# jonasrothfuss/meta_learning_pacoh

Hardware: AMD Instinct MI355X
Metric: task-GP LML+grad evals/sec (n_ctx=64, d=4, 20 particles) (higher is better)
Workload: dtype f32; 1 GPU; PACOH-SVGD step as meta_fit runs it (hipGraph replay), cfg#3: 1024 tasks per GPU x 20 particles, n_ctx=64, d=4, NN(32,32) mean + NN(32,32) kernel (D=2534), task sharding + 1 all-reduce/step; parallelism=task-shard x1, finite=True, tasks_total=1024, particles=20, n_ctx=64, d=4

## Files before the change

### include/pacoh_gp.h

```cpp
#ifndef PACOH_GP_H
#define PACOH_GP_H

#include <stddef.h>
#include <stdint.h>

#ifdef __cplusplus
extern "C" {
#endif

#define PACOH_F32 0
#define PACOH_F64 1

#define PACOH_OK 0
#define PACOH_EINVAL (-1)
#define PACOH_ELIMIT (-2)
#define PACOH_EDTYPE (-3)
#define PACOH_ELAUNCH (-4)

#define PACOH_MEAN_ZERO 0
#define PACOH_MEAN_VECTOR 1
#define PACOH_MEAN_CONST 2

#define PACOH_MAX_FEATURES 16
#define PACOH_KERNEL_RBF 0
// ... 218 lines not shown
                           int bandwidth_ready, int dtype, void* stream);

typedef struct pacoh_active_tasks {
    const int32_t* n_act;
    const void* task_w;
} pacoh_active_tasks;
typedef struct pacoh_active_feed {
    const int32_t* nact_all;
    const void* mult_all;
    int32_t* n_act; void* task_w;
} pacoh_active_feed;
int pacoh_mlp2_fwd_active(const pacoh_active_tasks* act, const void* x, int x_div, const void* theta, long theta_stride, int P, int d_in,
                          const int32_t* hidden, int n_hidden, long off_a, int d_out_a, void* out_a, long off_b, int d_out_b,
                          void* out_b, void* workspace, void* stash, int B, int n, int dtype, void* stream);
int pacoh_mlp2_fwd_svgd_active(const pacoh_active_tasks* act, const void* x, int x_div, const void* theta, long theta_stride, int P,
                               int d_in, const int32_t* hidden, int n_hidden, long off_a, int d_out_a, void* out_a, long off_b,
                               int d_out_b, void* out_b, void* workspace, void* stash, int B, int n,
                               const void* svgd_X, void* svgd_workspace, int svgd_P, int svgd_D, int64_t* counter,
                               int dtype, void* stream);
int pacoh_gp_lml_fwdbwd_active(const pacoh_active_tasks* act, const void* z, int z_div, const void* mean, int mean_mode,
                               const void* y, int y_div, const void* lengthscale, const void* outputscale,
                               const void* noise, const int32_t* n_valid, const void* g_lml,
                               void* lml, void* d_z, void* d_mean, void* d_lengthscale,
                               void* d_outputscale, void* d_noise, int32_t* info,
                               int B, int P, int n, int f, int dtype, void* stream);
int pacoh_mlp2_bwd_hyper_active(const pacoh_active_tasks* act, const void* x, int x_div, const void* theta, long theta_stride, int P,
                                int d_in, const int32_t* hidden, int n_hidden, long off_a, int d_out_a, const void* g_a, long off_b,
                                int d_out_b, const void* g_b, void* d_theta, long d_theta_stride, int accumulate,
                                void* workspace, const void* stash, int B, int n,
                                int T, int off_ls, int f, int off_os, int off_noise, int off_const, const void* d_lengthscale,
                                const void* d_outputscale, const void* d_noise, const void* d_const, const void* lml, void* lik,
                                double lik_scale, const int32_t* info, int32_t* fail_flag, void* svgd_workspace, int svgd_P, int svgd_D,
                                const pacoh_adam_inline* opt, int dtype, void* stream);
int pacoh_step_begin_active(const pacoh_active_feed* feed, const int64_t* idx_all, int tb, const void* sc_all, int n_sc,
                            const void* aux_all, long n_aux, int64_t* counter, int32_t* ticket, void* sc_out, void* aux_out,
                            const void* x, const void* y, const int32_t* n_valid, void* out_x, void* out_y, int32_t* out_n_valid, int n, int d,
                            const void* theta, long theta_stride, int P, int off_ls, int f, int off_os, int off_noise, double noise_floor,
                            void* ls, void* os, void* noise, int advance, const void* svgd_X, void* svgd_workspace, int svgd_P, int svgd_D,
                            int dtype, void* stream);
int pacoh_svgd_update_next_active(const pacoh_active_feed* feed, void* X, const void* score, const void* prior_mean, const void* prior_std,
                                  double prior_factor, double bandwidth, int use_adam, double beta1, double beta2, void* exp_avg,
                                  void* exp_avg_sq, void* bw_out, void* workspace, int P, int D,
                                  const int64_t* counter, void* sc2, int n_sc, const int64_t* idx_all, int tb, const void* sc_all,
                                  const void* x, const void* y, const int32_t* n_valid, void* out_x, void* out_y,
                                  int32_t* out_n_valid, int n, int d,
                                  int off_ls, int f, int off_os, int off_noise, double noise_floor, void* ls, void* os, void* noise,
                                  int bandwidth_ready, int dtype, void* stream);
#define PACOH_DECLINED 1
#define PACOH_DISTINCT_MAX_DRAWS 4096
#define PACOH_DISTINCT_MAX_TASKS 8192
int pacoh_distinct_rows(const int64_t* idx, int64_t* rows, void* mult, int32_t* n_act, int k, int tb, int n_tasks, int dtype,
                        void* stream);
int pacoh_mlp_fused_split(int tiles_eff, int tiles_full, int wgs, int tpw_host);
int pacoh_mlp_fused_plan(int R, int P, int nets, int n_hidden, int bwd, int resident, int* tile_points, int* wgs, int* tiles_per_wg);

size_t pacoh_svgd_imq_workspace_bytes(int P, int D, int dtype);
int pacoh_svgd_phi_imq(const void* X, const void* score, double alpha, double beta, double bandwidth,
                       int neg, void* phi, void* h_out, void* workspace, int P, int D, int dtype,
                       void* stream);

int pacoh_adam_step(void* param, const void* grad, void* exp_avg, void* exp_avg_sq,
                    double lr, double beta1, double beta2, double eps, double weight_decay,
                    long step, long count, int dtype, void* stream);

int pacoh_adam_step_dev(void* param, const void* grad, void* exp_avg, void* exp_avg_sq, const void* scalars,
                        double beta1, double beta2, long count, int64_t* step_counter, void* loss_cum, const void* loss,
                        int dtype, void* stream);

size_t pacoh_vi_update_dev_workspace_bytes(int D, int dtype);
int pacoh_vi_update_dev(void* posterior, const void* eps, const void* theta, const void* score, const void* lik,
                        const void* log_q, const void* prior_mean, const void* prior_std, double prior_factor,
                        const void* scalars, double beta1, double beta2, void* exp_avg, void* exp_avg_sq, void* loss_out,
                        int64_t* step_counter, void* workspace, int S, int D, int dtype, void* stream);

int pacoh_axpy(void* y, const void* x, double alpha, long count, int dtype, void* stream);

int pacoh_vi_sample(const void* posterior, const void* eps, void* theta, void* log_q, int S, int D, int dtype, void* stream);
int pacoh_vi_grad(const void* posterior, const void* eps, const void* score, double prior_factor, void* grad,
                  int S, int D, int dtype, void* stream);

int pacoh_vi_sample_full(const void* posterior, const void* eps, void* theta, void* log_q, int S, int D, int dtype,
                         void* stream);
int pacoh_vi_grad_full(const void* posterior, const void* eps, const void* score, double prior_factor, void* grad,
                       int S, int D, int dtype, void* stream);

int pacoh_gather_tasks(const void* x, const void* y, const int32_t* n_valid, const int64_t* idx, void* out_x,
                       void* out_y, int32_t* out_n_valid, int Tb, int n, int d, int dtype, void* stream);

int pacoh_reduce_tasks(const void* in, void* out, double scale, int accumulate, int T, int P, int W,
                       int dtype, void* stream);

#define PACOH_MAX_QUANTILES 2048

int pacoh_mixture_cdf(const void* mu, const void* var, const void* value, void* cdf, double y_mean, double y_std, int T, int P,
                      int m, int dtype, void* stream);
int pacoh_mixture_icdf(const void* mu, const void* var, const void* quantile, void* out, double y_mean, double y_std, double lo,
                       double hi, double eps, int max_iter, int closed_form, int P, int m, int dtype, void* stream);
int pacoh_calib_error(const void* cdf, void* out, int T, int m, int dtype, void* stream);

size_t pacoh_mvn_factor_workspace_bytes(int B, int m, int dtype);
int pacoh_mvn_factor(const void* cov, void* L, int32_t* info, void* workspace, int B, int m, int dtype, void* stream);
int pacoh_mvn_sample(const void* L, const int32_t* info, const void* mu, const void* eps, const int32_t* order,
                     const int32_t* offsets, void* out, double y_mean, double y_std, int B, int m, int S, int dtype, void* stream);

int pacoh_map_persist_supported(int n, int d, int tb, int mean_mode, const int32_t* mean_hidden, int n_mean_hidden, int kernel_nn,
                                const int32_t* kernel_hidden, int n_kernel_hidden, int f, int dtype);
// ... 45 lines not shown
```

### meta_learning_pacoh_amd/_lib.py

```python
import ctypes
import os

import torch

_HERE = os.path.dirname(os.path.abspath(__file__))
LIB_PATH = os.environ.get('PACOH_LIB') or os.path.join(_HERE, 'lib', 'libpacoh_gp.so')

F32, F64 = 0, 1
MEAN_ZERO, MEAN_VECTOR, MEAN_CONST = 0, 1, 2
KERNEL_RBF, KERNEL_COSINE, KERNEL_SHIFT = 0, 1, 8
KERNEL_MATERN12, KERNEL_MATERN32, KERNEL_MATERN52 = 3, 4, 5


def _kf(f, kernel):
    return int(f) | (int(kernel) << KERNEL_SHIFT)
ERRORS = {-1: 'PACOH_EINVAL (bad argument)', -2: 'PACOH_ELIMIT (shape outside kernel limits)',
          -3: 'PACOH_EDTYPE', -4: 'PACOH_ELAUNCH (HIP launch failed)', -5: 'PACOH_ENOCOMM (librccl not loadable)'}
COMM_ID_BYTES = 128

_c = ctypes
_vp, _i, _l, _d, _sz = _c.c_void_p, _c.c_int, _c.c_long, _c.c_double, _c.c_size_t
_ip = _c.POINTER(_c.c_int32)

SIGNATURES = {
# ... 49 lines not shown
    'pacoh_step_select': (_i, [_vp, _i, _vp, _i, _vp, _l, _vp, _vp, _vp, _vp, _i, _vp]),
    'pacoh_scale_dev': (_i, [_vp, _vp, _l, _i, _vp]),
    'pacoh_distinct_rows': (_i, [_vp, _vp, _vp, _vp, _i, _i, _i, _i, _vp]),
    'pacoh_step_begin': (_i, [_vp, _i, _vp, _i, _vp, _l, _vp, _vp, _vp, _vp, _vp, _vp, _vp, _vp, _vp, _vp, _i, _i,
                              _vp, _l, _i, _i, _i, _i, _i, _d, _vp, _vp, _vp, _i, _vp, _vp, _i, _i, _i, _vp]),
    'pacoh_step_begin_vi': (_i, [_vp, _i, _vp, _i, _vp, _l, _vp, _vp, _vp, _vp, _vp, _vp, _vp, _vp, _vp, _vp, _i, _i,
                                 _vp, _i, _i, _vp, _vp, _i, _i, _i, _i, _d, _vp, _vp, _vp, _i, _i, _vp]),
    'pacoh_svgd_update_dev_workspace_bytes': (_sz, [_i, _i, _i]),
    'pacoh_svgd_update_dev': (_i, [_vp, _vp, _vp, _vp, _d, _d, _i, _vp, _d, _d, _vp, _vp, _vp, _vp, _i, _i, _i, _vp, _i, _vp]),
    'pacoh_svgd_dist_advance': (_i, [_vp, _vp, _i, _i, _vp, _i, _vp]),
    'pacoh_svgd_update_next': (_i, [_vp, _vp, _vp, _vp, _d, _d, _i, _d, _d, _vp, _vp, _vp, _vp, _i, _i,
                                    _vp, _vp, _i, _vp, _i, _vp, _vp, _vp, _vp, _vp, _vp, _vp, _i, _i,
                                    _i, _i, _i, _i, _d, _vp, _vp, _vp, _i, _i, _vp]),
    'pacoh_prior_logprob_grad': (_i, [_vp, _vp, _vp, _vp, _vp, _d, _i, _i, _i, _vp]),
    'pacoh_prior_score_dev': (_i, [_vp, _vp, _vp, _vp, _d, _vp, _i, _i, _i, _vp]),
    'pacoh_svgd_workspace_bytes': (_sz, [_i, _i, _i]),
    'pacoh_svgd_phi': (_i, [_vp, _vp, _d, _i, _vp, _vp, _vp, _i, _i, _i, _vp]),
    'pacoh_svgd_update': (_i, [_vp, _vp, _vp, _vp, _d, _d, _i, _d, _d, _d, _d, _l, _vp, _vp, _vp, _vp, _vp, _i, _i, _i, _vp]),
    'pacoh_svgd_imq_workspace_bytes': (_sz, [_i, _i, _i]),
    'pacoh_svgd_phi_imq': (_i, [_vp, _vp, _d, _d, _d, _i, _vp, _vp, _vp, _i, _i, _i, _vp]),
    'pacoh_adam_step': (_i, [_vp, _vp, _vp, _vp, _d, _d, _d, _d, _d, _l, _l, _i, _vp]),
    'pacoh_adam_step_dev': (_i, [_vp, _vp, _vp, _vp, _vp, _d, _d, _l, _vp, _vp, _vp, _i, _vp]),
    'pacoh_vi_update_dev_workspace_bytes': (_sz, [_i, _i]),
    'pacoh_vi_update_dev': (_i, [_vp, _vp, _vp, _vp, _vp, _vp, _vp, _vp, _d, _vp, _d, _d, _vp, _vp, _vp, _vp, _vp, _i, _i, _i, _vp]),
    'pacoh_axpy': (_i, [_vp, _vp, _d, _l, _i, _vp]),
    'pacoh_vi_sample': (_i, [_vp, _vp, _vp, _vp, _i, _i, _i, _vp]),
    'pacoh_vi_grad': (_i, [_vp, _vp, _vp, _d, _vp, _i, _i, _i, _vp]),
    'pacoh_vi_sample_full': (_i, [_vp, _vp, _vp, _vp, _i, _i, _i, _vp]),
    'pacoh_vi_grad_full': (_i, [_vp, _vp, _vp, _d, _vp, _i, _i, _i, _vp]),
    'pacoh_gather_tasks': (_i, [_vp, _vp, _vp, _vp, _vp, _vp, _vp, _i, _i, _i, _i, _vp]),
    'pacoh_reduce_tasks': (_i, [_vp, _vp, _d, _i, _i, _i, _i, _i, _vp]),
    'pacoh_mixture_cdf': (_i, [_vp, _vp, _vp, _vp, _d, _d, _i, _i, _i, _i, _vp]),
    'pacoh_mixture_icdf': (_i, [_vp, _vp, _vp, _vp, _d, _d, _d, _d, _d, _i, _i, _i, _i, _i, _vp]),
    'pacoh_calib_error': (_i, [_vp, _vp, _i, _i, _i, _vp]),
    'pacoh_mvn_factor_workspace_bytes': (_sz, [_i, _i, _i]),
    'pacoh_mvn_factor': (_i, [_vp, _vp, _vp, _vp, _i, _i, _i, _vp]),
    'pacoh_mvn_sample': (_i, [_vp, _vp, _vp, _vp, _vp, _vp, _vp, _d, _d, _i, _i, _i, _i, _vp]),
    'pacoh_map_persist_supported': (_i, [_i, _i, _i, _i, _ip, _i, _i, _ip, _i, _i, _i]),
    'pacoh_map_persist': (_i, [_vp, _vp, _vp, _i, _vp, _vp, _vp, _i, _i, _vp, _i, _vp, _i, _i, _i, _i, _ip, _i, _i, _i, _ip, _i, _i,
                               _i, _i, _i, _d, _ip, _ip, _i, _d, _d, _vp, _vp, _vp, _i, _vp]),
    'pacoh_map_task_workspace_bytes': (_sz, [_i, _i, _i, _i, _i, _ip, _i, _i, _ip, _i, _i, _i, _i]),
    'pacoh_map_task_setup': (_i, [_vp, _i, _i, _i, _i, _i, _i, _ip, _i, _i, _i, _ip, _i, _i, _vp, _sz, _i, _vp]),
    'pacoh_svgd_task_workspace_bytes': (_sz, [_i, _i, _i, _i, _i, _i, _ip, _i, _i, _ip, _i, _i, _i, _i]),
    'pacoh_svgd_task_setup': (_i, [_i, _i, _i, _i, _i, _i, _i, _ip, _i, _i, _i, _ip, _i, _i, _vp, _sz, _i, _vp]),
    'pacoh_svgd_task_step': (_i, [_vp, _l, _i, _vp, _vp, _vp, _i, _i, _i, _i, _i, _ip, _i, _i, _i, _ip, _i, _i, _vp, _vp, _vp, _i, _i, _i,
                                  _vp, _l, _vp, _d, _vp, _vp, _sz, _vp, _vp, _i, _vp, _i, _i, _vp]),
    'pacoh_map_task_step': (_i, [_vp, _l, _vp, _vp, _vp, _i, _i, _i, _i, _i, _ip, _i, _i, _i, _ip, _i, _i, _vp, _vp, _vp, _i, _i, _i,
                                 _vp, _l, _vp, _d, _vp, _vp, _sz, _vp, _i, _vp]),
    'pacoh_comm_unique_id': (_i, [_vp]),
    'pacoh_comm_init': (_i, [_vp, _i, _i, _c.POINTER(_vp)]),
    'pacoh_allreduce_sum': (_i, [_vp, _l, _i, _vp, _vp]),
    'pacoh_comm_destroy': (_i, [_vp]),
    'pacoh_mlp_fused_split': (_i, [_i, _i, _i, _i]),
    'pacoh_mlp_fused_plan': (_i, [_i, _i, _i, _i, _i, _i, _ip, _ip, _ip]),
}
for _name in ('pacoh_mlp2_fwd', 'pacoh_mlp2_fwd_svgd', 'pacoh_gp_lml_fwdbwd', 'pacoh_mlp2_bwd_hyper', 'pacoh_step_begin',
              'pacoh_svgd_update_next'):
    SIGNATURES[_name + '_active'] = (_i, [_vp] + SIGNATURES[_name][1])

_lib = None
ABI_VERSION = 14


def load_library():
    global _lib
    if _lib is None:
        if not os.path.exists(LIB_PATH):
            raise RuntimeError(
                'libpacoh_gp.so not found at %s -- build it with `python -c "import __graft_entry__ as g; '
                'g.build()"` (needs hipcc). There is no CPU fallback for the PACOH GP path.' % LIB_PATH)
        lib = ctypes.CDLL(LIB_PATH)
        for name, (res, args) in SIGNATURES.items():
            if not hasattr(lib, name):
                raise RuntimeError('libpacoh_gp.so does not export %s (stale build?)' % name)
            fn = getattr(lib, name)
            fn.restype, fn.argtypes = res, args
        if lib.pacoh_abi_version() != ABI_VERSION:
            raise RuntimeError('%s has ABI version %d, this binding expects %d (stale build?)'
                               % (LIB_PATH, lib.pacoh_abi_version(), ABI_VERSION))
        _lib = lib
    return _lib


class ActiveTasks(ctypes.Structure):
    _fields_ = [('n_act', _vp), ('task_w', _vp)]


class ActiveFeed(ctypes.Structure):
    _fields_ = [('nact_all', _vp), ('mult_all', _vp), ('n_act', _vp), ('task_w', _vp)]


def _active_tasks(active):
    if active is None:
        return None
    n_act, task_w = active
    assert n_act.dtype == torch.int32 and n_act.is_cuda and task_w.is_cuda
    return ActiveTasks(n_act.data_ptr(), task_w.data_ptr())


def _active_feed(feed):
    if not getattr(feed, 'dedup', False):
        return None
    return ActiveFeed(feed.nact_all.data_ptr(), feed.mult_all.data_ptr(), feed.nact.data_ptr(), feed.mult.data_ptr())


def _active_call(lib, name, act, *args):
# ... 1334 lines not shown
```

### meta_learning_pacoh_amd/csrc/mlp_fused.hip

```cpp
#include "common.h"
#include "hyper_tail.h"
#include "step_tail.h"
#include "mlp_fused_split.h"
#include <stdlib.h>

namespace pacoh {

using f32x4 = __attribute__((ext_vector_type(4))) float;

constexpr int FMAXNH = 4;
constexpr int LWH = 36;
constexpr int HBLK = 32 * LWH + 32;
constexpr int F_OFF_W1 = 0;
constexpr int F_OFF_B1 = 128;
constexpr int F_OFF_H = 160;
__host__ __device__ constexpr int f_off_out(int nh) { return F_OFF_H + (nh - 1) * HBLK; }
__host__ __device__ constexpr int f_welems(int nh) { return f_off_out(nh) + 68; }
__host__ __device__ constexpr int f_dnet_max(int nh) { return 32 * 5 + (nh - 1) * 32 * 33 + 2 * 33; }
__host__ __device__ constexpr bool bwd_wg_slab(int nh) { return nh <= 2; }
constexpr int TSTRIDE = 4;
constexpr int TSTAGE = 6;
constexpr int TLD = 17;
__host__ __device__ constexpr int tskew(int k) { return 12 * (k & 1) + 32 * (k >> 1); }
constexpr int TRS = 320;

struct FusedNet {
    long theta_off;
    float* out;
    const float* g_out;
    float* slab;
    float* stash;
    int d_out, D_net;
};

struct FusedArgs {
    const float* x; int x_div;
    const float* theta; long theta_stride;
    FusedNet net[2];
    int P, n, R;
    int d_in, nh;
    int h[FMAXNH];
    int tiles_per_wg;
    int n_stash;
    int nblk;
    int tail_z;
    SvgdDistTail<float> sv;
    const float* bw_d2; float* bw_out; int bw_P;
    long* adv_counter;
    const int32_t* n_act;
    int tiles;
};

__device__ __forceinline__ void fused_live_rows(const FusedArgs& a, int tp, int& R, int& tpw) {
    R = a.R; tpw = a.tiles_per_wg;
    if (!a.n_act) return;
    const int live = *a.n_act * a.n;
    if (live < R) R = live;
    tpw = fused_split_tiles((R + tp - 1) / tp, a.tiles, (int)gridDim.x, tpw);
}

__device__ __forceinline__ long stash_off(const FusedArgs& a, int p, int blk, int slot, int fb, int lane) {
    return (((((long)p * a.nblk + blk) * a.n_stash + slot) * 2 + fb) << 8) + (lane << 2);
}

__device__ __forceinline__ f32x4 fmfma(float a, float b, f32x4 c) {
    return __builtin_amdgcn_mfma_f32_16x16x4f32(a, b, c, 0, 0, 0);
}

constexpr float TSC = 2.8853900817779268f, INV_TSC = 0.34657359027997264f;
__device__ __forceinline__ float tanh_pre(float a) {
    return fmaf(-2.0f, __builtin_amdgcn_rcpf(1.0f + __builtin_amdgcn_exp2f(a)), 1.0f);
}

template <int NH>
__device__ void fused_load_weights(float* wl, const float* __restrict__ th, const FusedArgs& a, int d_out) {
    for (int q = threadIdx.x; q < f_welems(NH); q += blockDim.x) wl[q] = 0.0f;
    __syncthreads();
    int src = 0;
    const int h0 = a.h[0], d_in = a.d_in;
    for (int q = threadIdx.x; q < h0; q += blockDim.x) wl[F_OFF_B1 + q] = TSC * th[q];
    for (int q = threadIdx.x; q < h0 * d_in; q += blockDim.x) { const int o = q / d_in, k = q - o * d_in; wl[F_OFF_W1 + o * 4 + k] = TSC * th[h0 + q]; }
    src += h0 * (d_in + 1);
    int prev = h0;
#pragma unroll
    for (int l = 1; l < NH; ++l) {
        const int hl = a.h[l];
        float* dst = wl + F_OFF_H + (l - 1) * HBLK;
        for (int q = threadIdx.x; q < hl; q += blockDim.x) dst[32 * LWH + q] = TSC * th[src + q];
        for (int q = threadIdx.x; q < hl * prev; q += blockDim.x) { const int o = q / prev, k = q - o * prev; dst[o * LWH + k] = TSC * th[src + hl + q]; }
        src += hl * (prev + 1);
        prev = hl;
    }
    float* dst = wl + f_off_out(NH);
    for (int q = threadIdx.x; q < d_out; q += blockDim.x) dst[64 + q] = th[src + q];
    for (int q = threadIdx.x; q < d_out * prev; q += blockDim.x) { const int o = q / prev, k = q - o * prev; dst[o * 32 + k] = th[src + d_out + q]; }
    __syncthreads();
}

template <int PB, bool BWD>
__device__ __forceinline__ long stage_tile(const FusedArgs& a, const FusedNet& nt, int p, int row0, float* st, int lane, int R) {
    long orow = -1;
    if (lane < 16 * PB) {
        const int row = row0 + lane;
        const bool valid = row < R;
        const int rr = valid ? row : R - 1;
        const int t = (int)((unsigned)rr / (unsigned)a.n), i = rr - t * a.n;
        const int bi = t * a.P + p;
        const int xb = a.x_div == 1 ? bi : (int)((unsigned)bi / (unsigned)a.x_div);
        const float* xq = a.x + ((long)xb * a.n + i) * (long)a.d_in;
        float4 xv;
        xv.x = xq[0];
        xv.y = a.d_in > 1 ? xq[1] : 0.0f;
        xv.z = a.d_in > 2 ? xq[2] : 0.0f;
        xv.w = a.d_in > 3 ? xq[3] : 0.0f;
        *reinterpret_cast<float4*>(st + lane * TSTRIDE) = xv;
        const long o = (long)bi * a.n + i;
        if (BWD) {
            const float* gq = nt.g_out + o * nt.d_out;
            st[16 * PB * TSTRIDE + lane] = valid ? gq[0] : 0.0f;
            st[16 * PB * (TSTRIDE + 1) + lane] = (valid && nt.d_out > 1) ? gq[1] : 0.0f;
        }
        orow = valid ? o : -1;
    }
    asm volatile("" ::: "memory");
    return orow;
}

template <int PB>
__device__ __forceinline__ void f_layer1(const float* wl, const float* st, int r, int g, f32x4 (&H)[2][PB]) {
    float bx[PB];
#pragma unroll
    for (int pb = 0; pb < PB; ++pb) bx[pb] = st[(pb * 16 + r) * TSTRIDE + g];
#pragma unroll
    for (int fb = 0; fb < 2; ++fb) {
        f32x4 bias;
#pragma unroll
        for (int s = 0; s < 4; ++s) bias[s] = wl[F_OFF_B1 + fb * 16 + 4 * g + s];
        const float aw = wl[F_OFF_W1 + (fb * 16 + r) * 4 + g];
#pragma unroll
        for (int pb = 0; pb < PB; ++pb) {
            f32x4 acc = fmfma(aw, bx[pb], bias);
#pragma unroll
            for (int s = 0; s < 4; ++s) acc[s] = tanh_pre(acc[s]);
            H[fb][pb] = acc;
        }
    }
}

template <int PB>
__device__ __forceinline__ void f_hidden(const float* W, int r, int g, const f32x4 (&IN)[2][PB], f32x4 (&OUT)[2][PB]) {
#pragma unroll
    for (int ob = 0; ob < 2; ++ob) {
        f32x4 bias;
#pragma unroll
        for (int s = 0; s < 4; ++s) bias[s] = W[32 * LWH + ob * 16 + 4 * g + s];
#pragma unroll
        for (int pb = 0; pb < PB; ++pb) OUT[ob][pb] = bias;
#pragma unroll
        for (int kb = 0; kb < 2; ++kb) {
            const float4 aw = *reinterpret_cast<const float4*>(W + (ob * 16 + r) * LWH + kb * 16 + 4 * g);
#pragma unroll
            for (int pb = 0; pb < PB; ++pb) {
                f32x4 acc = OUT[ob][pb];
                acc = fmfma(aw.x, IN[kb][pb][0], acc); acc = fmfma(aw.y, IN[kb][pb][1], acc);
                acc = fmfma(aw.z, IN[kb][pb][2], acc); acc = fmfma(aw.w, IN[kb][pb][3], acc);
                OUT[ob][pb] = acc;
            }
        }
#pragma unroll
        for (int pb = 0; pb < PB; ++pb)
#pragma unroll
            for (int s = 0; s < 4; ++s) OUT[ob][pb][s] = tanh_pre(OUT[ob][pb][s]);
    }
}

template <int PB>
__device__ __forceinline__ void f_delta(const float* W, int r, int g, const f32x4 (&DOUT)[2][PB], f32x4 (&HIN)[2][PB]) {
#pragma unroll
// ... 22 lines not shown
    f32x4 o;
#pragma unroll
    for (int s = 0; s < 4; ++s) scr[wr + s * TLD] = v[s];
    asm volatile("" ::: "memory");
#pragma unroll
    for (int q = 0; q < 4; ++q) o[q] = scr[rd + q];
    asm volatile("" ::: "memory");
    return o;
}

__device__ __forceinline__ void f_wgrad(f32x4& acc, const f32x4& Ap, const f32x4& Bp) {
    acc = fmfma(Ap[0], Bp[0], acc); acc = fmfma(Ap[1], Bp[1], acc);
    acc = fmfma(Ap[2], Bp[2], acc); acc = fmfma(Ap[3], Bp[3], acc);
}

__device__ __forceinline__ void stash_st(const f32x4& v, f32x4* q) {
    __builtin_nontemporal_store(v, q);
}
__device__ __forceinline__ f32x4 stash_ld(const f32x4* q) {
    return *q;
}

template <int PB>
__device__ __forceinline__ void stash_put(const FusedArgs& a, const FusedNet& nt, int p, int blk0, int slot, int lane,
                                          const f32x4 (&H)[2][PB]) {
#pragma unroll
    for (int pb = 0; pb < PB; ++pb)
#pragma unroll
        for (int fb = 0; fb < 2; ++fb)
            stash_st(H[fb][pb], reinterpret_cast<f32x4*>(nt.stash + stash_off(a, p, blk0 + pb, slot, fb, lane)));
}

template <int PB>
__device__ __forceinline__ void stash_get(const FusedArgs& a, const FusedNet& nt, int p, int blk0, int slot, int lane,
                                          f32x4 (&H)[2][PB], int R) {
#pragma unroll
    for (int pb = 0; pb < PB; ++pb) {
        const bool in = (blk0 + pb) * 16 < R;
#pragma unroll
        for (int fb = 0; fb < 2; ++fb)
            H[fb][pb] = in ? stash_ld(reinterpret_cast<const f32x4*>(nt.stash + stash_off(a, p, blk0 + pb, slot, fb, lane)))
                           : f32x4{0.f, 0.f, 0.f, 0.f};
    }
}

template <int NH, int PB, int MINW>
__global__ void __launch_bounds__(256, MINW) mlp_fused_fwd_kernel(FusedArgs a) {
    __shared__ __attribute__((aligned(16))) float wl[f_welems(NH)];
    __shared__ __attribute__((aligned(16))) float stage[4][16 * PB * TSTAGE];
    if (a.tail_z > 0 && (int)blockIdx.z == a.tail_z) {
        svgd_dist_tail<float>(a.sv, (int)(blockIdx.y * gridDim.x + blockIdx.x), (int)(gridDim.x * gridDim.y));
        return;
    }
    int R, tpw;
    fused_live_rows(a, 16 * PB, R, tpw);
    const FusedNet& nt = a.net[blockIdx.z];
    const int p = blockIdx.y;
    fused_load_weights<NH>(wl, a.theta + (long)p * a.theta_stride + nt.theta_off, a, nt.d_out);
    const int lane = threadIdx.x & 63, wave = __builtin_amdgcn_readfirstlane(threadIdx.x >> 6);
    const int r = lane & 15, g = lane >> 4;
    float* st = stage[wave];
    const float* wo = wl + f_off_out(NH);
    float w3r[2][2][4];
#pragma unroll
    for (int o = 0; o < 2; ++o)
#pragma unroll
        for (int fb = 0; fb < 2; ++fb)
#pragma unroll
            for (int s = 0; s < 4; ++s) w3r[o][fb][s] = wo[o * 32 + fb * 16 + 4 * g + s];
    const float b30 = wo[64], b31 = wo[65];
    constexpr int TP = 16 * PB;
    for (int tl = wave; tl < tpw; tl += 4) {
        const int row0 = (blockIdx.x * tpw + tl) * TP;
        if (row0 >= R) break;
        const long orow_l = stage_tile<PB, false>(a, nt, p, row0, st, lane, R);
        f32x4 HA[2][PB], HB[2][PB];
        const int blk0 = row0 >> 4;
        const int ns = nt.stash ? a.n_stash : 0;
        f_layer1<PB>(wl, st, r, g, HA);
        if (ns >= NH) stash_put<PB>(a, nt, p, blk0, 0, lane, HA);
#pragma unroll
        for (int l = 1; l < NH; ++l) {
            if (l & 1) f_hidden<PB>(wl + F_OFF_H + (l - 1) * HBLK, r, g, HA, HB);
            else f_hidden<PB>(wl + F_OFF_H + (l - 1) * HBLK, r, g, HB, HA);
            if (l >= NH - ns) stash_put<PB>(a, nt, p, blk0, l - (NH - ns), lane, (l & 1) ? HB : HA);
        }
        const f32x4 (&HL)[2][PB] = ((NH - 1) & 1) ? HB : HA;
#pragma unroll
        for (int pb = 0; pb < PB; ++pb) {
            float v0 = 0.f, v1 = 0.f;
#pragma unroll
            for (int fb = 0; fb < 2; ++fb)
#pragma unroll
                for (int s = 0; s < 4; ++s) { v0 = fmaf(w3r[0][fb][s], HL[fb][pb][s], v0); v1 = fmaf(w3r[1][fb][s], HL[fb][pb][s], v1); }
            v0 += __shfl_xor(v0, 16, 64); v0 += __shfl_xor(v0, 32, 64);
            v1 += __shfl_xor(v1, 16, 64); v1 += __shfl_xor(v1, 32, 64);
            const long orow = __shfl(orow_l, pb * 16 + r, 64);
            if (g == 0 && orow >= 0) {
                nt.out[orow * nt.d_out] = v0 + b30;
                if (nt.d_out > 1) nt.out[orow * nt.d_out + 1] = v1 + b31;
            }
        }
    }
}

template <int NH, int PB, int MINW>
__global__ void __launch_bounds__(256, MINW) mlp_fused_bwd_kernel(FusedArgs a) {
    constexpr int L_WL = (f_welems(NH) + 3) & ~3, L_ST = 4 * 16 * PB * TSTAGE, L_TS = 4 * 2 * TRS;
    constexpr int L_RED = bwd_wg_slab(NH) ? 4 * f_dnet_max(NH) : 0;
    constexpr int L_ALL = (L_WL + L_ST + L_TS) > L_RED ? (L_WL + L_ST + L_TS) : L_RED;
    __shared__ __attribute__((aligned(16))) float lds[L_ALL];
    if (a.tail_z > 0 && (int)blockIdx.z == a.tail_z) {
        if (blockIdx.x == 0 && blockIdx.y == 0) {
            if (a.bw_out) svgd_bandwidth_block<float>(a.bw_d2, a.bw_P, a.bw_out);
            if (a.adv_counter && threadIdx.x == 0) *a.adv_counter += 1;
        }
        return;
    }
    int R, tpw;
    fused_live_rows(a, 16 * PB, R, tpw);
    float* wl = lds;
    const FusedNet& nt = a.net[blockIdx.z];
    const int p = blockIdx.y;
    fused_load_weights<NH>(wl, a.theta + (long)p * a.theta_stride + nt.theta_off, a, nt.d_out);
    const int lane = threadIdx.x & 63, wave = __builtin_amdgcn_readfirstlane(threadIdx.x >> 6);
    const int r = lane & 15, g = lane >> 4;
    float* st = lds + L_WL + wave * (16 * PB * TSTAGE);
    float* sc0 = lds + L_WL + L_ST + wave * (2 * TRS);
    float* sc1 = sc0 + TRS;
    const int twr = 4 * TLD * g + tskew(g) + r, trd = TLD * r + tskew(r >> 2) + 4 * g;
    const float* wo = wl + f_off_out(NH);

    f32x4 aW[NH > 1 ? NH - 1 : 1][2][2] = {};
    float aBh[NH > 1 ? NH - 1 : 1][2] = {};
    float aW1[2][4] = {}, aB1[2] = {};
    f32x4 aWoT[2][2] = {};
    float aBoT[2] = {};

    constexpr int TP = 16 * PB;
    for (int tl = wave; tl < tpw; tl += 4) {
        const int row0 = (blockIdx.x * tpw + tl) * TP;
        if (row0 >= R) break;
        stage_tile<PB, true>(a, nt, p, row0, st, lane, R);
        f32x4 H[NH][2][PB];
        const int blk0 = row0 >> 4;
        const int ns = nt.stash ? a.n_stash : 0;
#pragma unroll
        for (int l = NH - 1; l >= 0; --l)
            if (l >= NH - ns) stash_get<PB>(a, nt, p, blk0, l - (NH - ns), lane, H[l], R);
        if (ns < NH) f_layer1<PB>(wl, st, r, g, H[0]);
#pragma unroll
        for (int l = 1; l < NH; ++l)
            if (l < NH - ns) f_hidden<PB>(wl + F_OFF_H + (l - 1) * HBLK, r, g, H[l - 1], H[l]);
        {
// ... 181 lines not shown
    return (tiles + best_tpw - 1) / best_tpw;
}

static int fused_n_stash(int n_hidden) { return n_hidden > 1 ? n_hidden - 1 : 0; }
static int fused_nblk(int B, int P, int n) { return 4 * (int)(((long)(B / P) * n + 63) / 64); }

size_t mlp_fused_stash_bytes(int B, int P, int n, int n_hidden, int nets) {
    return (size_t)nets * P * fused_nblk(B, P, n) * fused_n_stash(n_hidden) * 2 * 256 * sizeof(float);
}

static void fused_fill(FusedArgs& a, const void* x, int x_div, const void* theta, long theta_stride, int P, int d_in,
                       const int32_t* hidden, int n_hidden, int B, int n, const void* stash, int nets) {
    a.x = (const float*)x; a.x_div = x_div; a.theta = (const float*)theta; a.theta_stride = theta_stride;
    a.P = P; a.n = n; a.R = (B / P) * n; a.d_in = d_in; a.nh = n_hidden;
    for (int l = 0; l < FMAXNH; ++l) a.h[l] = l < n_hidden ? hidden[l] : 0;
    a.n_stash = stash ? fused_n_stash(n_hidden) : 0;
    a.nblk = fused_nblk(B, P, n);
    const size_t per_net = (size_t)P * a.nblk * a.n_stash * 2 * 256;
    for (int k = 0; k < 2; ++k) a.net[k].stash = (a.n_stash > 0 && k < nets) ? (float*)stash + k * per_net : nullptr;
}

static int fused_fwd_tpw(int tiles, int P, int nets) {
    int pick = 4;
    double best = 1e30;
    for (int tpw = 4; tpw <= 32; tpw *= 2) {
        const long waves = (long)((tiles + tpw - 1) / tpw) * P * nets * 4;
        const double cost = (double)((waves + 1023) / 1024) * (tpw / 4 + 0.5);
        if (cost <= best * 1.02 || tpw == 4) { if (cost < best) best = cost; pick = tpw; }
    }
    return pick;
}

constexpr int BWD_MINW = 3;
constexpr int BWD_MINW_PB2 = 2;
#define PACOH_FUSED_DISPATCH(KERNEL, nh, pb, M)                                                          \
    do {                                                                                                 \
        if (pb == 4) {                                                                                   \
            if (nh == 1) { M((KERNEL<1, 4, BWD_MINW>)); } else if (nh == 2) { M((KERNEL<2, 4, BWD_MINW>)); }  \
            else if (nh == 3) { M((KERNEL<3, 4, 1>)); } else { M((KERNEL<4, 4, 1>)); }                    \
        } else {                                                                                         \
            if (nh == 1) { M((KERNEL<1, 2, BWD_MINW_PB2>)); } else if (nh == 2) { M((KERNEL<2, 2, BWD_MINW_PB2>)); }            \
            else if (nh == 3) { M((KERNEL<3, 2, 2>)); } else { M((KERNEL<4, 2, 2>)); }                    \
        }                                                                                                \
    } while (0)

int mlp_fused_fwd(const void* x, int x_div, const void* theta, long theta_stride, int P, int d_in, const int32_t* hidden,
                  int n_hidden, int nets, const long* off, const int* d_out, void* const* out, void* stash, int B, int n,
                  hipStream_t s, const SvgdDistTail<float>* tail, bool* tail_taken, const int32_t* n_act) {
    FusedArgs a = {};
    fused_fill(a, x, x_div, theta, theta_stride, P, d_in, hidden, n_hidden, B, n, stash, nets);
    for (int k = 0; k < nets; ++k) { a.net[k].theta_off = off[k]; a.net[k].out = (float*)out[k]; a.net[k].d_out = d_out[k]; }
    const int pb = fused_fwd_pb(a.R, P, nets);
    const int tiles = (a.R + 16 * pb - 1) / (16 * pb);
    a.n_act = n_act; a.tiles = tiles;
    a.tiles_per_wg = fused_fwd_tpw(tiles, P, nets);
    const int wgs = (tiles + a.tiles_per_wg - 1) / a.tiles_per_wg;
    if (tail && (long)wgs * P * 2 < (long)tail->P * (tail->P + 1) / 2) tail = nullptr;
    if (tail_taken) *tail_taken = tail != nullptr;
    if (tail) { a.tail_z = nets; a.sv = *tail; }
#define PACOH_LAUNCH_FWD(K) hipLaunchKernelGGL((K), dim3(wgs, P, nets + (tail ? 1 : 0)), dim3(256), 0, s, a)
    if (pb == 4) {
        if (n_hidden == 1) PACOH_LAUNCH_FWD((mlp_fused_fwd_kernel<1, 4, 4>)); else if (n_hidden == 2) PACOH_LAUNCH_FWD((mlp_fused_fwd_kernel<2, 4, 4>));
        else if (n_hidden == 3) PACOH_LAUNCH_FWD((mlp_fused_fwd_kernel<3, 4, 4>)); else PACOH_LAUNCH_FWD((mlp_fused_fwd_kernel<4, 4, 4>));
    } else {
        if (n_hidden == 1) PACOH_LAUNCH_FWD((mlp_fused_fwd_kernel<1, 2, 4>)); else if (n_hidden == 2) PACOH_LAUNCH_FWD((mlp_fused_fwd_kernel<2, 2, 4>));
        else if (n_hidden == 3) PACOH_LAUNCH_FWD((mlp_fused_fwd_kernel<3, 2, 4>)); else PACOH_LAUNCH_FWD((mlp_fused_fwd_kernel<4, 2, 4>));
    }
#undef PACOH_LAUNCH_FWD
    return launch_status();
}

struct FusedBwdPlan { int pb, chunks, tiles_per_wg; };

static FusedBwdPlan fused_bwd_plan(int R, int P, int nets, int n_hidden, int resident_given = 0) {
    FusedBwdPlan pl;
    pl.pb = fused_bwd_pb(n_hidden, R, P, nets);
    static int resident[FMAXNH + 1][2] = {};
    int res = resident_given;
    if (res <= 0) {
        int& cached = resident[n_hidden][pl.pb == 4];
        if (cached == 0) {
#define PACOH_OCC(K) cached = resident_wgs(K)
            PACOH_FUSED_DISPATCH(mlp_fused_bwd_kernel, n_hidden, pl.pb, PACOH_OCC);
#undef PACOH_OCC
        }
        res = cached;
    }
    const int tp = 16 * pl.pb;
    pl.chunks = fused_chunks(R, P, nets, tp, res, 0.4 * 64 / tp);
    const int tiles = (R + tp - 1) / tp;
    pl.tiles_per_wg = (tiles + pl.chunks - 1) / pl.chunks;
    return pl;
}

size_t mlp_fused_bwd_workspace(int B, int P, int n, int d_in, const int32_t* hidden, int n_hidden, int d_out, int nets) {
    const FusedBwdPlan pl = fused_bwd_plan((B / P) * n, P, nets, n_hidden);
    return (size_t)pl.chunks * (bwd_wg_slab(n_hidden) ? 1 : 4) * P * fused_dnet(d_in, hidden, n_hidden, d_out) * sizeof(float);
}

int mlp_fused_bwd(const void* x, int x_div, const void* theta, long theta_stride, int P, int d_in, const int32_t* hidden,
                  int n_hidden, int nets, const long* off, const int* d_out, const void* const* g_out, void* d_theta,
                  long d_theta_stride, int accumulate, void* workspace, const void* stash, int B, int n, hipStream_t s,
                  const HyperBwdArgs<float>* tail, long col_base) {
    FusedArgs a = {};
    fused_fill(a, x, x_div, theta, theta_stride, P, d_in, hidden, n_hidden, B, n, stash, nets);
    const FusedBwdPlan pl = fused_bwd_plan(a.R, P, nets, n_hidden);
    a.tiles_per_wg = pl.tiles_per_wg;
    a.n_act = tail ? tail->n_act : nullptr; a.tiles = (a.R + 16 * pl.pb - 1) / (16 * pl.pb);
    float* ws = (float*)workspace;
    SlabReduce sr[2] = {};
    int wmax = 0;
    for (int k = 0; k < nets; ++k) {
        a.net[k].theta_off = off[k]; a.net[k].g_out = (const float*)g_out[k]; a.net[k].d_out = d_out[k];
        a.net[k].D_net = fused_dnet(d_in, hidden, n_hidden, d_out[k]);
        a.net[k].slab = ws;
        sr[k].in = ws; sr[k].out = (float*)d_theta + off[k]; sr[k].Wd = a.net[k].D_net; sr[k].col0 = (int)(col_base + off[k]);
        ws += (size_t)pl.chunks * (bwd_wg_slab(n_hidden) ? 1 : 4) * P * a.net[k].D_net;
        if (a.net[k].D_net > wmax) wmax = a.net[k].D_net;
    }
    HyperBwdArgs<float> rtail = tail ? *tail : HyperBwdArgs<float>{};
    const bool bw_here = tail && tail->sv_bw, adv_here = tail && tail->nx.counter;
    if (bw_here) { a.bw_d2 = tail->sv_d2; a.bw_P = tail->sv_P; a.bw_out = tail->sv_bw; rtail.sv_bw = nullptr; }
    if (adv_here) a.adv_counter = const_cast<long*>(tail->nx.counter);
    if (bw_here || adv_here) a.tail_z = nets;
#define PACOH_LAUNCH_BWD(K) hipLaunchKernelGGL(K, dim3(pl.chunks, P, nets + ((bw_here || adv_here) ? 1 : 0)), dim3(256), 0, s, a)
    PACOH_FUSED_DISPATCH(mlp_fused_bwd_kernel, n_hidden, pl.pb, PACOH_LAUNCH_BWD);
#undef PACOH_LAUNCH_BWD
    const long tot = (long)P * wmax;
    unsigned gx = (unsigned)((tot * 8 + 255) / 256);
    const int tail_blocks = tail ? hyper_tail_blocks(rtail) : 0;
    if ((unsigned)tail_blocks > gx) gx = (unsigned)tail_blocks;
    hipLaunchKernelGGL(fused_reduce_slab_kernel<3>, dim3(gx, nets + (tail ? 1 : 0)), dim3(256), 0, s,
                       sr[0], sr[1], d_theta_stride, accumulate, pl.chunks * (bwd_wg_slab(n_hidden) ? 1 : 4), P, nets,
                       rtail, tail_blocks, (float*)nullptr, (const int*)nullptr);
    return launch_status();
}

}

extern "C" int pacoh_mlp_fused_split(int tiles_eff, int tiles_full, int wgs, int tpw_host) {
    return pacoh::fused_split_tiles(tiles_eff, tiles_full, wgs, tpw_host);
}
extern "C" int pacoh_mlp_fused_plan(int R, int P, int nets, int n_hidden, int bwd, int resident, int* tile_points, int* wgs, int* tiles_per_wg) {
    using namespace pacoh;
    if (R <= 0 || P <= 0 || nets < 1 || nets > 2 || n_hidden < 1 || n_hidden > FMAXNH || !tile_points || !wgs || !tiles_per_wg) return PACOH_EINVAL;
    if (bwd) {
        const FusedBwdPlan pl = fused_bwd_plan(R, P, nets, n_hidden, resident);
        *tile_points = 16 * pl.pb; *wgs = pl.chunks; *tiles_per_wg = pl.tiles_per_wg;
    } else {
        const int pb = fused_fwd_pb(R, P, nets);
        *tile_points = 16 * pb;
        *tiles_per_wg = fused_fwd_tpw((R + 16 * pb - 1) / (16 * pb), P, nets);
        *wgs = ((R + 16 * pb - 1) / (16 * pb) + *tiles_per_wg - 1) / *tiles_per_wg;
    }
    return PACOH_OK;
}

namespace pacoh {

int fused_reduce_launch(const float* slab0, int wd0, long off0, const float* slab1, int wd1, long off1, int nets, float* d_theta,
                        long d_theta_stride, int slabs, const HyperBwdArgs<float>* tail, float* img_th, const int* img_map, hipStream_t s, int P) {
    SlabReduce sr[2] = {{slab0, d_theta + off0, wd0, (int)off0}, {slab1, d_theta + off1, wd1, (int)off1}};
    const int wmax = wd0 > wd1 ? wd0 : wd1;
    const int lsh = slabs <= 2 ? 1 : (slabs <= 16 ? 3 : 5);
    unsigned gx = (unsigned)((((long)P * wmax << lsh) + 255) / 256);
    const int tail_blocks = tail ? hyper_tail_blocks(*tail) : 0;
    if ((unsigned)tail_blocks > gx) gx = (unsigned)tail_blocks;
#define PACOH_REDUCE(LSH) hipLaunchKernelGGL(fused_reduce_slab_kernel<LSH>, dim3(gx, nets + (tail ? 1 : 0)), dim3(256), 0, s, sr[0], sr[1], \
                                             d_theta_stride, 0, slabs, P, nets, tail ? *tail : HyperBwdArgs<float>{}, tail_blocks, img_th, img_map)
    if (lsh == 1) PACOH_REDUCE(1); else if (lsh == 3) PACOH_REDUCE(3); else PACOH_REDUCE(5);
#undef PACOH_REDUCE
    return launch_status();
}

}
```

### meta_learning_pacoh_amd/csrc/mlp_fused_split.h

```cpp
#pragma once

namespace pacoh {

__host__ __device__ inline int fused_split_tiles(int tiles_eff, int tiles_full, int wgs, int tpw_host) {
    if (tiles_eff >= tiles_full) return tpw_host;
    const int share = ((tiles_eff + wgs - 1) / wgs + 3) & ~3;
    return share < tpw_host ? share : tpw_host;
}

}
```

Measured before the change: 68.12 million evals/s.

## Interleave forward MLP tiles across workgroups and use permlane swaps for output reduction

The fused MLP forward kernel now assigns tiles round-robin across workgroups and waves, replacing contiguous per-workgroup chunks. Workgroups with no live tile exit before loading weights. When only some tasks are active, this spreads the live rows evenly across the grid instead of piling them onto the first workgroups. The output reduction swaps xor-shuffles for permlane16/32 swap builtins, so each lane group writes one output column and no shuffle of the row index is needed. Output row indices are stashed in LDS during staging, and the permlane builtins tie the code to hardware that supports them.

```diff
diff --git a/include/pacoh_gp.h b/include/pacoh_gp.h
--- a/include/pacoh_gp.h
+++ b/include/pacoh_gp.h
@@ -294,6 +294,7 @@
 int pacoh_distinct_rows(const int64_t* idx, int64_t* rows, void* mult, int32_t* n_act, int k, int tb, int n_tasks, int dtype,
                         void* stream);
 int pacoh_mlp_fused_split(int tiles_eff, int tiles_full, int wgs, int tpw_host);
+int pacoh_mlp_fused_fwd_tile(int wgs, int wg, int wave, int k);
 int pacoh_mlp_fused_plan(int R, int P, int nets, int n_hidden, int bwd, int resident, int* tile_points, int* wgs, int* tiles_per_wg);
 
 size_t pacoh_svgd_imq_workspace_bytes(int P, int D, int dtype);
diff --git a/meta_learning_pacoh_amd/_lib.py b/meta_learning_pacoh_amd/_lib.py
--- a/meta_learning_pacoh_amd/_lib.py
+++ b/meta_learning_pacoh_amd/_lib.py
@@ -125,6 +125,7 @@
     'pacoh_allreduce_sum': (_i, [_vp, _l, _i, _vp, _vp]),
     'pacoh_comm_destroy': (_i, [_vp]),
     'pacoh_mlp_fused_split': (_i, [_i, _i, _i, _i]),
+    'pacoh_mlp_fused_fwd_tile': (_i, [_i, _i, _i, _i]),
     'pacoh_mlp_fused_plan': (_i, [_i, _i, _i, _i, _i, _i, _ip, _ip, _ip]),
 }
 for _name in ('pacoh_mlp2_fwd', 'pacoh_mlp2_fwd_svgd', 'pacoh_gp_lml_fwdbwd', 'pacoh_mlp2_bwd_hyper', 'pacoh_step_begin',
diff --git a/meta_learning_pacoh_amd/csrc/mlp_fused.hip b/meta_learning_pacoh_amd/csrc/mlp_fused.hip
--- a/meta_learning_pacoh_amd/csrc/mlp_fused.hip
+++ b/meta_learning_pacoh_amd/csrc/mlp_fused.hip
@@ -51,12 +51,15 @@
     int tiles;
 };
 
+__device__ __forceinline__ int fused_live_R(const FusedArgs& a) {
+    if (!a.n_act) return a.R;
+    const int live = *a.n_act * a.n;
+    return live < a.R ? live : a.R;
+}
+
 __device__ __forceinline__ void fused_live_rows(const FusedArgs& a, int tp, int& R, int& tpw) {
-    R = a.R; tpw = a.tiles_per_wg;
-    if (!a.n_act) return;
-    const int live = *a.n_act * a.n;
-    if (live < R) R = live;
-    tpw = fused_split_tiles((R + tp - 1) / tp, a.tiles, (int)gridDim.x, tpw);
+    R = fused_live_R(a); tpw = a.tiles_per_wg;
+    if (a.n_act) tpw = fused_split_tiles((R + tp - 1) / tp, a.tiles, (int)gridDim.x, tpw);
 }
 
 __device__ __forceinline__ long stash_off(const FusedArgs& a, int p, int blk, int slot, int fb, int lane) {
@@ -98,8 +101,7 @@
 }
 
 template <int PB, bool BWD>
-__device__ __forceinline__ long stage_tile(const FusedArgs& a, const FusedNet& nt, int p, int row0, float* st, int lane, int R) {
-    long orow = -1;
+__device__ __forceinline__ void stage_tile(const FusedArgs& a, const FusedNet& nt, int p, int row0, float* st, int lane, int R) {
     if (lane < 16 * PB) {
         const int row = row0 + lane;
         const bool valid = row < R;
@@ -119,11 +121,16 @@
             const float* gq = nt.g_out + o * nt.d_out;
             st[16 * PB * TSTRIDE + lane] = valid ? gq[0] : 0.0f;
             st[16 * PB * (TSTRIDE + 1) + lane] = (valid && nt.d_out > 1) ? gq[1] : 0.0f;
-        }
-        orow = valid ? o : -1;
+        } else {
+            reinterpret_cast<long*>(st + 16 * PB * TSTRIDE)[lane] = valid ? o : -1;
+        }
     }
     asm volatile("" ::: "memory");
-    return orow;
+}
+
+template <int PB>
+__device__ __forceinline__ long f_out_row(const float* st, int pt) {
+    return reinterpret_cast<const long*>(st + 16 * PB * TSTRIDE)[pt];
 }
 
 template <int PB>
@@ -252,8 +259,10 @@
         svgd_dist_tail<float>(a.sv, (int)(blockIdx.y * gridDim.x + blockIdx.x), (int)(gridDim.x * gridDim.y));
         return;
     }
-    int R, tpw;
-    fused_live_rows(a, 16 * PB, R, tpw);
+    constexpr int TP = 16 * PB;
+    const int R = fused_live_R(a);
+    const int tiles_eff = (R + TP - 1) / TP, wgs = (int)gridDim.x;
+    if (fused_fwd_tile(wgs, (int)blockIdx.x, 0, 0) >= tiles_eff) return;
     const FusedNet& nt = a.net[blockIdx.z];
     const int p = blockIdx.y;
     fused_load_weights<NH>(wl, a.theta + (long)p * a.theta_stride + nt.theta_off, a, nt.d_out);
@@ -268,12 +277,14 @@
         for (int fb = 0; fb < 2; ++fb)
 #pragma unroll
             for (int s = 0; s < 4; ++s) w3r[o][fb][s] = wo[o * 32 + fb * 16 + 4 * g + s];
-    const float b30 = wo[64], b31 = wo[65];
-    constexpr int TP = 16 * PB;
-    for (int tl = wave; tl < tpw; tl += 4) {
-        const int row0 = (blockIdx.x * tpw + tl) * TP;
-        if (row0 >= R) break;
-        const long orow_l = stage_tile<PB, false>(a, nt, p, row0, st, lane, R);
+    const float bo = wo[64 + (g & 1)];
+    float* const out = nt.out;
+    const int d_out = nt.d_out;
+    for (int k = 0;; ++k) {
+        const int tile = fused_fwd_tile(wgs, (int)blockIdx.x, wave, k);
+        if (tile >= tiles_eff) break;
+        const int row0 = tile * TP;
+        stage_tile<PB, false>(a, nt, p, row0, st, lane, R);
         f32x4 HA[2][PB], HB[2][PB];
         const int blk0 = row0 >> 4;
         const int ns = nt.stash ? a.n_stash : 0;
@@ -286,6 +297,9 @@
             if (l >= NH - ns) stash_put<PB>(a, nt, p, blk0, l - (NH - ns), lane, (l & 1) ? HB : HA);
         }
         const f32x4 (&HL)[2][PB] = ((NH - 1) & 1) ? HB : HA;
+        long orow[PB];
+#pragma unroll
+        for (int pb = 0; pb < PB; ++pb) { const long o = f_out_row<PB>(st, pb * 16 + r); orow[pb] = g < d_out ? o : -1; }
 #pragma unroll
         for (int pb = 0; pb < PB; ++pb) {
             float v0 = 0.f, v1 = 0.f;
@@ -293,13 +307,11 @@
             for (int fb = 0; fb < 2; ++fb)
 #pragma unroll
                 for (int s = 0; s < 4; ++s) { v0 = fmaf(w3r[0][fb][s], HL[fb][pb][s], v0); v1 = fmaf(w3r[1][fb][s], HL[fb][pb][s], v1); }
-            v0 += __shfl_xor(v0, 16, 64); v0 += __shfl_xor(v0, 32, 64);
-            v1 += __shfl_xor(v1, 16, 64); v1 += __shfl_xor(v1, 32, 64);
-            const long orow = __shfl(orow_l, pb * 16 + r, 64);
-            if (g == 0 && orow >= 0) {
-                nt.out[orow * nt.d_out] = v0 + b30;
-                if (nt.d_out > 1) nt.out[orow * nt.d_out + 1] = v1 + b31;
-            }
+            const auto h = __builtin_amdgcn_permlane16_swap(__float_as_uint(v0), __float_as_uint(v1), false, false);
+            const unsigned s = __float_as_uint(__uint_as_float(h[0]) + __uint_as_float(h[1]));
+            const auto w = __builtin_amdgcn_permlane32_swap(s, s, false, false);
+            const float tot = __uint_as_float(w[0]) + __uint_as_float(w[1]);
+            if (orow[pb] >= 0) out[orow[pb] * d_out + g] = tot + bo;
         }
     }
 }
@@ -587,9 +599,9 @@
     for (int k = 0; k < nets; ++k) { a.net[k].theta_off = off[k]; a.net[k].out = (float*)out[k]; a.net[k].d_out = d_out[k]; }
     const int pb = fused_fwd_pb(a.R, P, nets);
     const int tiles = (a.R + 16 * pb - 1) / (16 * pb);
-    a.n_act = n_act; a.tiles = tiles;
-    a.tiles_per_wg = fused_fwd_tpw(tiles, P, nets);
-    const int wgs = (tiles + a.tiles_per_wg - 1) / a.tiles_per_wg;
+    a.n_act = n_act;
+    const int tpw = fused_fwd_tpw(tiles, P, nets);
+    const int wgs = (tiles + tpw - 1) / tpw;
     if (tail && (long)wgs * P * 2 < (long)tail->P * (tail->P + 1) / 2) tail = nullptr;
     if (tail_taken) *tail_taken = tail != nullptr;
     if (tail) { a.tail_z = nets; a.sv = *tail; }
@@ -676,6 +688,7 @@
 extern "C" int pacoh_mlp_fused_split(int tiles_eff, int tiles_full, int wgs, int tpw_host) {
     return pacoh::fused_split_tiles(tiles_eff, tiles_full, wgs, tpw_host);
 }
+extern "C" int pacoh_mlp_fused_fwd_tile(int wgs, int wg, int wave, int k) { return pacoh::fused_fwd_tile(wgs, wg, wave, k); }
 extern "C" int pacoh_mlp_fused_plan(int R, int P, int nets, int n_hidden, int bwd, int resident, int* tile_points, int* wgs, int* tiles_per_wg) {
     using namespace pacoh;
     if (R <= 0 || P <= 0 || nets < 1 || nets > 2 || n_hidden < 1 || n_hidden > FMAXNH || !tile_points || !wgs || !tiles_per_wg) return PACOH_EINVAL;
diff --git a/meta_learning_pacoh_amd/csrc/mlp_fused_split.h b/meta_learning_pacoh_amd/csrc/mlp_fused_split.h
--- a/meta_learning_pacoh_amd/csrc/mlp_fused_split.h
+++ b/meta_learning_pacoh_amd/csrc/mlp_fused_split.h
@@ -1,6 +1,8 @@
 #pragma once
 
 namespace pacoh {
+
+__host__ __device__ inline int fused_fwd_tile(int wgs, int wg, int wave, int k) { return (k * wgs + wg) * 4 + wave; }
 
 __host__ __device__ inline int fused_split_tiles(int tiles_eff, int tiles_full, int wgs, int tpw_host) {
     if (tiles_eff >= tiles_full) return tpw_host;
```

Result: no change. 68.65 million evals/s, median of 6 (+0.8%).
